# WeebLabs/DSPi

Hardware: AMD Instinct MI355X
Metric: audio samples/s (whole node), 96 kHz 11-ch 10-band PEQ; % HBM roofline (higher is better)
Workload: dtype f32

## Files before the change

dspi_amd/csrc/dspi_capi.cpp:

```cpp
#include <hip/hip_runtime.h>

#include <string.h>

#include <memory>
#include <new>
#include <cstdlib>
#include <string>
#include <unordered_map>
#include <type_traits>
#include <vector>
#include <thread>
#include <xmmintrin.h>
#include <algorithm>
#include <atomic>
#include <chrono>
#include "../../include/dspi_detmath.h"

#include "../../include/dspi.h"
#include "dspi_image.h"
#include "dspi_kernels.h"
#include "dspi_params.h"
#include "dspi_boot.h"
#include "dspi_move.h"
#include "dspi_plan.h"
#include "dspi_resize.h"
#include "dspi_snapshot.h"
#include "dspi_spdifpos.h"

using namespace dspi;

struct dspi_ctx {
    int flavor = 1;
    bool fma = false;
    uint32_t n_streams = 0, n_wg = 0;
    uint32_t cap_wg = 0;
    int device = DSPI_DEVICE_NONE;
    StateMap sm{};
    std::vector<std::unique_ptr<Params>> images;
    std::vector<uint32_t> image_refs;
    std::vector<int32_t> stream_image;
    bool assignment_dirty = true;
    bool merge_hint = false;
    std::vector<std::vector<WgItem>> image_rows;
    std::vector<uint32_t> image_rows_offset;
    PlanInput plan_in;
    LaunchPlan plan;
    WgItem *d_litems = nullptr; size_t d_litems_cap = 0;
    uint32_t *d_stream_image = nullptr; size_t d_stream_image_cap = 0;
    bool launch_dirty = true;
    uint32_t spdif_pos = 0;
    SpdifPos spdif_ps;
    uint32_t *d_spdif_ps = nullptr; size_t d_spdif_ps_cap = 0;
    uint32_t *d_spdif_vpos = nullptr; size_t d_spdif_vpos_cap = 0;
    bool populated = false;
    bool audio_started = false;
    bool no_direct = false;
    std::vector<uint32_t> lv_alphas; uint32_t lv_checked_count = 0; size_t lv_checked_n = 0;
    uint32_t direct_spin_us = 0;
    uint64_t direct_stats[5] = {0, 0, 0, 0, 0};
    hipStream_t hs = nullptr;
    hipStream_t hs_in = nullptr, hs_out = nullptr;
    std::vector<hipEvent_t> pipe_events;
    uint32_t *d_state = nullptr, *d_dlines = nullptr, *d_ring = nullptr;
    uint32_t *d_xwords = nullptr; size_t d_xwords_cap = 0;
    DevImage *d_images = nullptr;
    std::vector<uint32_t> image_flags;
    std::vector<uint8_t> image_touched;
    float *d_vals = nullptr; size_t d_vals_cap = 0;
    uint32_t *d_pv_rows = nullptr; size_t d_pv_rows_cap = 0;
    size_t d_images_cap = 0;
    WgItem *d_items = nullptr;
    size_t d_items_cap = 0;
    void *d_in = nullptr; size_t d_in_cap = 0;
    int32_t *d_pairs = nullptr; size_t d_pairs_cap = 0;
    int32_t *d_sub = nullptr; size_t d_sub_cap = 0;
    uint16_t *d_peaks = nullptr; size_t d_peaks_cap = 0;
    uint16_t *d_clip = nullptr; size_t d_clip_cap = 0;
    char *h_direct = nullptr; char *d_direct = nullptr; size_t direct_cap = 0;
    uint32_t *h_done = nullptr; uint32_t *d_done = nullptr; uint32_t direct_seq = 0; int direct_flag = -1;
    int32_t *d_spdif_words = nullptr; size_t d_spdif_words_cap = 0;
    uint32_t *d_pdm = nullptr;
    int32_t *d_pdm_in = nullptr; size_t d_pdm_in_cap = 0;
    uint32_t *d_pdm_out = nullptr; size_t d_pdm_out_cap = 0;
    int32_t *d_spdif_in = nullptr; size_t d_spdif_in_cap = 0;
    uint32_t *d_spdif_out = nullptr; size_t d_spdif_out_cap = 0;
    uint32_t *d_snap = nullptr; size_t d_snap_cap = 0;
    uint32_t *d_snap_shift = nullptr; size_t d_snap_shift_cap = 0;
    std::vector<uint8_t> active; uint32_t n_paused = 0;
    std::vector<std::pair<uint32_t, uint32_t>> paused_runs; bool paused_runs_dirty = false;
    uint32_t *d_active = nullptr; size_t d_active_cap = 0; bool active_dirty = false;
    uint32_t move_batch = 0;
    uint32_t *d_move = nullptr; size_t d_move_cap = 0;
    uint32_t *h_move = nullptr; size_t h_move_cap = 0; hipEvent_t ev_move = nullptr;
    std::string err;
};

namespace {

int fail(dspi_ctx *c, int code, const std::string &msg) { if (c) c->err = msg; return code; }

#define HIPCK(c, call)                                                                                   \
    do {                                                                                                 \
        hipError_t e_ = (call);                                                                          \
        if (e_ != hipSuccess) return fail((c), DSPI_E_HIP, std::string(#call) + ": " + hipGetErrorString(e_)); \
    } while (0)

bool valid_stream(const dspi_ctx *c, int32_t s) { return s == DSPI_ALL_STREAMS || (s >= 0 && (uint32_t)s < c->n_streams); }

int32_t add_image(dspi_ctx *c, std::unique_ptr<Params> p) {
// ... 332 lines not shown
    return 0;
}

int fetch_status(dspi_ctx *c, int32_t stream, uint16_t *peaks, uint16_t *clip) {
    for (int i = 0; i < kMaxCh; i++) peaks[i] = 0;
    *clip = 0;
    if (c->device == DSPI_DEVICE_NONE) return 0;
    const uint32_t s = stream == DSPI_ALL_STREAMS ? 0u : (uint32_t)stream;
    uint32_t w[kMaxCh + 4];
    int rc = read_stream_words(c, s, c->sm.peaks, c->sm.n_ch + 4, w);
    if (rc) return rc;
    for (int i = 0; i < c->sm.n_ch; i++) peaks[i] = (uint16_t)w[i];
    *clip = (uint16_t)(w[c->sm.n_ch] | w[c->sm.n_ch + 1] | w[c->sm.n_ch + 2] | w[c->sm.n_ch + 3]);
    return 0;
}

int zero_clips(dspi_ctx *c, int32_t stream) {
    if (c->device == DSPI_DEVICE_NONE) return 0;
    HIPCK(c, hipSetDevice(c->device));
    HIPCK(c, hipStreamSynchronize(c->hs));
    const size_t row = (size_t)c->sm.row, pitch = (size_t)c->sm.n_slots * row * 4;
    if (stream == DSPI_ALL_STREAMS) {
        HIPCK(c, hipMemset2D(c->d_state + (size_t)c->sm.clip * row, pitch, 0, 4 * row * 4, c->n_wg));
    } else {
        const uint32_t wg = (uint32_t)stream / (uint32_t)row, col = (uint32_t)stream % (uint32_t)row;
        uint32_t z[4] = {0, 0, 0, 0};
        HIPCK(c, hipMemcpy2D(c->d_state + ((size_t)wg * c->sm.n_slots + c->sm.clip) * row + col, row * 4, z, 4, 4, 4, hipMemcpyHostToDevice));
    }
    return 0;
}

}

extern "C" {

int dspi_abi_version(void) { return DSPI_ABI_VERSION; }

int dspi_create(dspi_ctx **out, int flavor, uint32_t n_streams, int hip_device) {
    const bool fma = (flavor & DSPI_FLOAT_CONTRACT_FMA) != 0, populated = (flavor & DSPI_BOOT_POPULATED_FLASH) != 0;
    flavor &= ~(DSPI_FLOAT_CONTRACT_FMA | DSPI_BOOT_POPULATED_FLASH);
    if (!out || (flavor != DSPI_FLAVOR_RP2040_Q28 && flavor != DSPI_FLAVOR_RP2350_F32) || n_streams == 0) return DSPI_E_INVAL;
    if (fma && flavor != DSPI_FLAVOR_RP2350_F32) return DSPI_E_INVAL;
    dspi_ctx *c = new (std::nothrow) dspi_ctx();
    if (!c) return DSPI_E_NOMEM;
    c->flavor = flavor;
    c->n_streams = n_streams;
    c->device = hip_device;
    c->sm = make_state_map(flavor);
    c->n_wg = (n_streams + (uint32_t)c->sm.row - 1) / (uint32_t)c->sm.row;
    c->cap_wg = c->n_wg;
    c->fma = fma;
    c->populated = populated;
    c->no_direct = getenv("DSPI_NO_DIRECT") != nullptr;
    if (const char *e = getenv("DSPI_DIRECT_SPIN_US")) { const long v = atol(e); if (v > 0) c->direct_spin_us = (uint32_t)std::min<long>(v, 1000000L); }
    if (const char *e = getenv("DSPI_MOVE_BATCH")) { const long v = atol(e); if (v > 0) c->move_batch = (uint32_t)std::min<long>(std::max<long>(v, 2L), 65535L); }
    c->images.push_back(std::make_unique<Params>(flavor, fma, !populated));
    c->image_refs.push_back(n_streams);
    c->stream_image.assign(n_streams, 0);
    *out = c;
    if (hip_device == DSPI_DEVICE_NONE) return DSPI_OK;

    int count = 0;
    if (hipGetDeviceCount(&count) != hipSuccess || count <= 0) { *out = nullptr; delete c; return DSPI_E_NODEVICE; }
    auto bail = [&](int code) { dspi_destroy(c); *out = nullptr; return code; };
    if (hipSetDevice(hip_device) != hipSuccess) return bail(DSPI_E_NODEVICE);
    if (hipStreamCreateWithFlags(&c->hs, hipStreamNonBlocking) != hipSuccess) return bail(DSPI_E_HIP);
    const size_t row = (size_t)c->sm.row;
    const size_t state_b = (size_t)c->n_wg * c->sm.n_slots * row * 4;
    const size_t dl_b = (size_t)c->n_wg * c->sm.n_out * (size_t)c->sm.max_delay * row * 4;
    const size_t ring_b = (size_t)c->n_wg * kRingLen * 2 * row * 4;
    if (hipMalloc((void **)&c->d_state, state_b) != hipSuccess || hipMalloc((void **)&c->d_dlines, dl_b) != hipSuccess ||
        hipMalloc((void **)&c->d_ring, ring_b) != hipSuccess)
        return bail(DSPI_E_NOMEM);
    if (hipMemsetAsync(c->d_state, 0, state_b, c->hs) != hipSuccess || hipMemsetAsync(c->d_dlines, 0, dl_b, c->hs) != hipSuccess ||
        hipMemsetAsync(c->d_ring, 0, ring_b, c->hs) != hipSuccess || launch_state_init(flavor, c->d_state, c->n_wg, c->hs) != hipSuccess ||
        hipStreamSynchronize(c->hs) != hipSuccess)
        return bail(DSPI_E_HIP);
    return DSPI_OK;
}

void dspi_destroy(dspi_ctx *c) {
    if (!c) return;
    if (c->device != DSPI_DEVICE_NONE) {
        (void)hipSetDevice(c->device);
        if (c->hs) (void)hipStreamSynchronize(c->hs);
        for (void *p : {(void *)c->d_state, (void *)c->d_dlines, (void *)c->d_ring, (void *)c->d_xwords, (void *)c->d_vals, (void *)c->d_pv_rows, (void *)c->d_images, (void *)c->d_items, (void *)c->d_litems, (void *)c->d_stream_image, (void *)c->d_pdm, (void *)c->d_pdm_in, (void *)c->d_pdm_out, (void *)c->d_spdif_in, (void *)c->d_spdif_out, (void *)c->d_spdif_ps, (void *)c->d_spdif_vpos, (void *)c->d_snap, (void *)c->d_snap_shift, (void *)c->d_active, (void *)c->d_move, c->d_in,
                        (void *)c->d_pairs, (void *)c->d_sub, (void *)c->d_peaks, (void *)c->d_clip, (void *)c->d_spdif_words})
            if (p) (void)hipFree(p);
        if (c->h_direct) (void)hipHostFree(c->h_direct);
        if (c->h_done) (void)hipHostFree(c->h_done);
        if (c->h_move) (void)hipHostFree(c->h_move);
        if (c->ev_move) (void)hipEventDestroy(c->ev_move);
        for (hipEvent_t e : c->pipe_events) (void)hipEventDestroy(e);
        if (c->hs_in) (void)hipStreamDestroy(c->hs_in);
        if (c->hs_out) (void)hipStreamDestroy(c->hs_out);
        if (c->hs) (void)hipStreamDestroy(c->hs);
    }
    delete c;
}

const char *dspi_last_error(const dspi_ctx *c) { return c ? c->err.c_str() : "null context"; }
int dspi_num_channels(const dspi_ctx *c) { return c ? c->sm.n_ch : DSPI_E_INVAL; }
int dspi_num_outputs(const dspi_ctx *c) { return c ? c->sm.n_out : DSPI_E_INVAL; }
int dspi_num_pairs(const dspi_ctx *c) { return c ? c->sm.n_pairs : DSPI_E_INVAL; }
uint32_t dspi_num_streams(const dspi_ctx *c) { return c ? c->n_streams : 0; }
uint32_t dspi_tile_streams(const dspi_ctx *c) { return c ? (uint32_t)c->sm.row : 0; }
// ... 57 lines not shown
        if (cap < 1) return DSPI_E_SHORT;
        const uint8_t slot = wValue & 0xFF, type = (wValue >> 8) & 0xFF;
        bool changes = false;
        for (size_t i = 0; i < c->images.size() && !changes; i++) {
            if (stream == DSPI_ALL_STREAMS ? c->image_refs[i] == 0 : (size_t)c->stream_image[(size_t)stream] != i) continue;
            const Params &r = *c->images[i];
            changes = slot < r.n_pairs && type <= 1 && type != r.output_types[slot];
        }
        if (!changes) { Params view = readable(c, stream); return view.vendor_get(req, wValue, buf, cap, peaks, &clip); }
    }
    if (req == 0xD6 || req == 0xC0) {
        return for_targets(c, stream, [&](Params &p) { int r = p.vendor_get(req, wValue, buf, cap, peaks, &clip); return r < 0 ? r : 0; }) == 0 ? 1 : DSPI_E_SHORT;
    }
    Params tmp_view = readable(c, stream);
    n = tmp_view.vendor_get(req, wValue, buf, cap, peaks, &clip);
    if (req == 0x83 && n >= 0 && (before != 0 || stream == DSPI_ALL_STREAMS)) { int rc = zero_clips(c, stream); if (rc) return rc; }
    return n;
}
int dspi_set_host_volume(dspi_ctx *c, int32_t stream, int16_t v) {
    return for_targets(c, stream, [&](Params &p) { p.set_volume(v); return 0; });
}
int dspi_set_mute(dspi_ctx *c, int32_t stream, int mute) {
    return for_targets(c, stream, [&](Params &p) { p.set_mute(mute != 0); return 0; });
}
int dspi_set_sample_rate(dspi_ctx *c, int32_t stream, uint32_t hz) {
    if (hz != 44100 && hz != 48000 && hz != 96000) return DSPI_E_INVAL;
    return for_targets(c, stream, [&](Params &p) { return p.set_rate(hz); });
}

int dspi_get_status(dspi_ctx *c, int32_t stream, void *buf, size_t cap) {
    if (!c || !buf || !valid_stream(c, stream)) return DSPI_E_INVAL;
    const int n = c->sm.n_ch * 2 + 4;
    if (cap < (size_t)n) return DSPI_E_SHORT;
    return dspi_vendor_get(c, stream, 0x50, 9, buf, (uint16_t)n);
}
int dspi_clear_clips(dspi_ctx *c, int32_t stream) {
    if (!c || !valid_stream(c, stream)) return DSPI_E_INVAL;
    uint16_t f = 0;
    int n = dspi_vendor_get(c, stream, 0x83, 0, &f, 2);
    return n < 0 ? n : (int)f;
}

int dspi_debug_image(dspi_ctx *c, int32_t stream, void *buf, size_t cap) {
    if (!c || !buf || !valid_stream(c, stream)) return DSPI_E_INVAL;
    if (cap < sizeof(DevImage)) return DSPI_E_SHORT;
    DevImage img;
    readable(c, stream).build_image(img);
    memcpy(buf, &img, sizeof(img));
    return (int)sizeof(img);
}

int dspi_debug_launch_plan(dspi_ctx *c, uint32_t *counts, size_t n_counts) {
    if (!c || !counts || n_counts < 5) return DSPI_E_INVAL;
    const int n = n_counts >= 7 ? 7 : n_counts >= 6 ? 6 : 5;
    uint32_t all[7] = {};
    for (const PathInfo &pi : kPaths) {
        const uint32_t k = (uint32_t)c->plan.items[(int)pi.path].size();
        all[(int)pi.group] += k;
        if (pi.paired) all[6] += k;
    }
    for (int k = 0; k < n; k++) counts[k] = all[k];
    return n;
}

int dspi_debug_direct_stats(dspi_ctx *c, uint64_t *out, size_t n) {
    if (!c || !out || n < 5) return DSPI_E_INVAL;
    for (int i = 0; i < 5; i++) out[i] = c->direct_stats[i];
    return 5;
}

int dspi_debug_image_count(dspi_ctx *c) {
    if (!c) return DSPI_E_INVAL;
    if (c->merge_hint) merge_images(c);
    return (int)c->images.size();
}

int dspi_debug_eq_taps(dspi_ctx *c, int32_t stream, int channel, const float *x, uint32_t n, float *taps, float *other) {
    if (!c || !x || !taps || !other || n == 0 || n > (1u << 20) || !valid_stream(c, stream) || stream < 0) return DSPI_E_INVAL;
    if (c->flavor != DSPI_FLAVOR_RP2350_F32 || channel < 0 || channel >= c->sm.n_ch) return DSPI_E_INVAL;
    if (c->device == DSPI_DEVICE_NONE) return fail(c, DSPI_E_NODEVICE, "host-only context: the HIP path is the only audio path");
    HIPCK(c, hipSetDevice(c->device));
    DevImage img;
    readable(c, stream).build_image(img);
    DevImage *d_img = nullptr; float *d_x = nullptr, *d_t = nullptr, *d_o = nullptr;
    const size_t nb = (size_t)n * sizeof(float);
    auto done = [&](int rc) { (void)hipFree(d_img); (void)hipFree(d_x); (void)hipFree(d_t); (void)hipFree(d_o); return rc; };
    if (hipMalloc((void **)&d_img, sizeof img) != hipSuccess || hipMalloc((void **)&d_x, nb) != hipSuccess ||
        hipMalloc((void **)&d_t, nb * (kBands + 1)) != hipSuccess || hipMalloc((void **)&d_o, nb * kBands) != hipSuccess)
        return done(fail(c, DSPI_E_NOMEM, "hipMalloc failed (EQ taps)"));
    if (hipMemcpy(d_img, &img, sizeof img, hipMemcpyHostToDevice) != hipSuccess || hipMemcpy(d_x, x, nb, hipMemcpyHostToDevice) != hipSuccess ||
        launch_eq_taps(c->fma, d_img, channel, d_x, n, d_t, d_o, c->hs) != hipSuccess || hipStreamSynchronize(c->hs) != hipSuccess ||
        hipMemcpy(taps, d_t, nb * (kBands + 1), hipMemcpyDeviceToHost) != hipSuccess || hipMemcpy(other, d_o, nb * kBands, hipMemcpyDeviceToHost) != hipSuccess)
        return done(fail(c, DSPI_E_HIP, "EQ taps failed"));
    return done(DSPI_OK);
}

int dspi_debug_detmath(dspi_ctx *c, int which, const float *a, const float *b, uint32_t n, float *out) {
    if (!c || !a || !out || ((which == 1 || which == 4) && !b) || n == 0 || n > (1u << 24) || which < 0 || which > 4) return DSPI_E_INVAL;
    if (c->device == DSPI_DEVICE_NONE) return fail(c, DSPI_E_NODEVICE, "host-only context: the HIP path is the only audio path");
    HIPCK(c, hipSetDevice(c->device));
    float *d_a = nullptr, *d_b = nullptr, *d_o = nullptr;
    const size_t nb = (size_t)n * sizeof(float);
    auto done = [&](int rc) { (void)hipFree(d_a); (void)hipFree(d_b); (void)hipFree(d_o); return rc; };
    if (hipMalloc((void **)&d_a, nb) != hipSuccess || hipMalloc((void **)&d_b, nb) != hipSuccess || hipMalloc((void **)&d_o, nb) != hipSuccess)
        return done(fail(c, DSPI_E_NOMEM, "hipMalloc failed (detmath)"));
    if (hipMemcpy(d_a, a, nb, hipMemcpyHostToDevice) != hipSuccess || hipMemcpy(d_b, (which == 1 || which == 4) ? b : a, nb, hipMemcpyHostToDevice) != hipSuccess ||
        launch_detmath(which, d_a, d_b, n, d_o, c->hs) != hipSuccess || hipStreamSynchronize(c->hs) != hipSuccess ||
        hipMemcpy(out, d_o, nb, hipMemcpyDeviceToHost) != hipSuccess)
// ... 796 lines not shown
            if ((he = hipEventRecord(c->pipe_events[2 * ch], sin)) != hipSuccess || (he = hipStreamWaitEvent(c->hs, c->pipe_events[2 * ch], 0)) != hipSuccess) return fail_hip(he, "event");
        }
        if ((rc = launch_rows(c, a, L, r0, r1))) { unpin(); return rc; }
        if (n_chunks > 1) {
            if ((he = hipEventRecord(c->pipe_events[2 * ch + 1], c->hs)) != hipSuccess || (he = hipStreamWaitEvent(sout, c->pipe_events[2 * ch + 1], 0)) != hipSuccess) return fail_hip(he, "event");
        }
        for (int k = 1; k < 4; k++)
            if (bufs[k].host && (he = copy(bufs[k], hipMemcpyDeviceToHost, sout)) != hipSuccess) return fail_hip(he, bufs[k].what);
    }
    if (clip_out) {
        if ((rc = gather_clip(c, c->d_clip))) { unpin(); return rc; }
        if ((he = hipMemcpyAsync(clip_out, c->d_clip, L.clip.bytes, hipMemcpyDeviceToHost, c->hs)) != hipSuccess) return fail_hip(he, "D2H clip flags");
    }
    if (n_chunks > 1) {
        if ((he = hipStreamSynchronize(c->hs_out)) != hipSuccess) return fail_hip(he, "sync");
        if ((he = hipStreamSynchronize(c->hs_in)) != hipSuccess) return fail_hip(he, "sync");
    }
    if ((he = hipStreamSynchronize(c->hs)) != hipSuccess) return fail_hip(he, "sync");
    unpin();
    return DSPI_OK;
}

int dspi_process(dspi_ctx *c, const void *pcm_in, int bit_depth, uint32_t n_blocks, uint32_t block_len, const dspi_out *out, uint32_t flags) {
    if (!c || !pcm_in || !out) return DSPI_E_INVAL;
    constexpr uint32_t kKnownFlags = DSPI_MEM_DEVICE | DSPI_OUT_TILED | DSPI_OUT_ENABLED_ONLY | DSPI_OUT_I2S_SLOTS | DSPI_OUT_SPDIF | DSPI_OUT_CLIP_FLAGS;
    if (flags & ~kKnownFlags) return fail(c, DSPI_E_INVAL, "dspi_process: undefined flag bits");
    if (c->device == DSPI_DEVICE_NONE) return fail(c, DSPI_E_NODEVICE, "host-only context: the HIP path is the only audio path");
    if ((bit_depth != 16 && bit_depth != 24) || n_blocks == 0 || block_len == 0 || block_len > DSPI_MAX_BLOCK_LEN)
        return fail(c, DSPI_E_INVAL, "bit_depth must be 16/24, 1 <= block_len <= 192, n_blocks >= 1");
    const auto call_t0 = std::chrono::steady_clock::now();
    HIPCK(c, hipSetDevice(c->device));
    int rc = commit_params(c);
    if (rc || (rc = check_leveller_alphas(c, block_len))) return rc;

    uint16_t *const clip_out = (flags & DSPI_OUT_CLIP_FLAGS) ? out->clip_flags : nullptr;
    CallInput in;
    in.n_streams = c->n_streams; in.n_wg = c->n_wg; in.row = (uint32_t)c->sm.row; in.n_ch = (uint32_t)c->sm.n_ch; in.n_out = (uint32_t)c->sm.n_out;
    in.n_pairs = (uint32_t)c->sm.n_pairs; in.n_blocks = n_blocks; in.block_len = block_len; in.bit_depth = (uint32_t)bit_depth; in.flags = flags;
    in.pairs = out->pairs; in.sub = out->sub; in.peaks = out->peaks; in.clip = clip_out; in.no_direct = c->no_direct;
    in.all_latency = c->flavor != 0; in.spdif_per_stream = c->spdif_ps.on;
    for (const PathInfo &pi : kPaths)
        if (pi.group != PathGroup::Latency && !c->plan.items[(int)pi.path].empty()) in.all_latency = false;
    const CallLayout L = plan_call(in);
    const bool tiled = flags & DSPI_OUT_TILED, spdif = flags & DSPI_OUT_SPDIF;
    if (spdif && (tiled || (flags & DSPI_OUT_I2S_SLOTS))) return fail(c, DSPI_E_INVAL, "DSPI_OUT_SPDIF goes with neither DSPI_OUT_TILED nor DSPI_OUT_I2S_SLOTS");
    if (L.spdif_two_pass && c->spdif_ps.on && (rc = upload_spdif_pos(c))) return rc;

    KArgs a{};
    a.img = c->d_images; a.stream_image = c->d_stream_image; a.vals = c->d_vals;
    a.state = c->d_state; a.dlines = c->d_dlines; a.ring = c->d_ring;
    a.n_streams = c->n_streams; a.n_blocks = n_blocks; a.block_len = block_len; a.bit_depth = (uint32_t)bit_depth;
    a.tiled_out = tiled ? 1u : 0u;
    a.fma = c->fma ? 1u : 0u;
    a.skip_silent = ((flags & DSPI_OUT_ENABLED_ONLY) && !L.spdif_two_pass) ? 1u : 0u;
    a.i2s_slots = (flags & DSPI_OUT_I2S_SLOTS) ? 1u : 0u;
    if (spdif) { a.spdif = L.spdif_two_pass ? 0u : 1u; a.spdif_pos = c->spdif_pos; }
    if (c->flavor && !tiled) {
        const size_t xb = (size_t)c->n_wg * 3 * kMaxOut * kChunk * c->sm.row * 4;
        if ((rc = ensure(c, c->d_xwords, c->d_xwords_cap, xb))) return rc;
        a.xwords = c->d_xwords;
    }

    switch (L.mem) {
    case CallMem::Device: rc = process_device(c, L, a, pcm_in, out, clip_out); break;
    case CallMem::Direct: rc = process_direct(c, L, a, pcm_in, out, clip_out, flags, call_t0); break;
    case CallMem::Staged: rc = process_staged(c, L, a, pcm_in, out, clip_out, flags); break;
    }
    if (rc == DSPI_OK && spdif) {
        c->spdif_pos = (uint32_t)((c->spdif_pos + L.frames) % 192u);
        if (c->spdif_ps.on) c->spdif_ps.advance(L.frames);
    }
    return rc;
}

}
```

dspi_amd/csrc/dspi_chain_pk.inc:

```

typedef float v2f __attribute__((ext_vector_type(2)));
typedef uint32_t v2u __attribute__((ext_vector_type(2)));

#ifndef DSPI_EXP_EMIT
#define DSPI_EXP_EMIT 0
#endif
#ifndef DSPI_EMIT_PAIRS
#define DSPI_EMIT_PAIRS 0xC
#endif
constexpr uint32_t ROWP = 128;
constexpr int HALF = 64;
constexpr int kMailbox = 8;

__device__ __forceinline__ v2f as_v2f(v2u u) { return __builtin_bit_cast(v2f, u); }
__device__ __forceinline__ v2u as_v2u(v2f f) { return __builtin_bit_cast(v2u, f); }
__device__ __forceinline__ v2f splat(float f) { return v2f{f, f}; }
__device__ __forceinline__ float clamp_pm1(float x) {
    float r;
    asm("v_med3_f32 %0, %1, -1.0, 1.0" : "=v"(r) : "v"(x));
    return r;
}
__device__ __forceinline__ float peak_acc(float pk, float x) { asm("v_max_f32 %0, |%1|, %0" : "+v"(pk) : "v"(x)); return pk; }
__device__ __forceinline__ float peak_acc2(float pk, float a, float b) { asm("v_max3_f32 %0, |%1|, |%2|, %0" : "+v"(pk) : "v"(a), "v"(b)); return pk; }

// ... 1002 lines not shown
    constexpr int P = make_state_map(1).n_pairs;
    const size_t F = (size_t)g.n_blocks * g.B;
    const int en = TAIL ? (int)min((uint32_t)T, g.B - e_cq * T) : T;
    uint32_t stream_ = stream, lane_ = lane;
    asm volatile("" : "+v"(stream_), "+v"(lane_));
    if (e_cq == 0) { pk[0] = splat(0.0f); pk[1] = splat(0.0f); }
#pragma unroll
    for (int side = 0; side < 2; ++side)
#pragma unroll
        for (int i = 0; i < T; i += 2) {
            const v2f y0 = live(dl[side][i], TAIL, i, en), y1 = live(dl[side][i + 1], TAIL, i + 1, en);
            pk[side].x = peak_acc2(pk[side].x, y0.x, y1.x);
            pk[side].y = peak_acc2(pk[side].y, y0.y, y1.y);
        }
    if (e_cq == g.cpb - 1) {
#pragma unroll
        for (int side = 0; side < 2; ++side) {
            const int oo = 2 * p + side;
            v2u p16;
#pragma unroll
            for (int c = 0; c < 2; ++c) {
                p16[c] = (uint32_t)(fminf(1.0f, pk[side][c]) * 32767.0f);
                if (pk[side][c] > 1.001f) clip[c] |= 1u << (2 + oo);
                if (a.peaks) a.peaks[((size_t)(stream_ + c) * g.n_blocks + e_kq) * sm.n_ch + 2 + oo] = (uint16_t)p16[c];
            }
            if (e_kq == g.n_blocks - 1) *reinterpret_cast<v2u *>(a.state + ((size_t)wg * sm.n_slots + sm.peaks + 2 + oo) * ROWP + lane_ * 2) = p16;
        }
    }
    if (a.pairs) {
        const float scale = ((img->out_enabled >> (2 * p)) & 3u) ? 8388607.0f : 0.0f;
        const bool shift = a.i2s_slots && ((img->i2s_pairs >> p) & 1u);
        int32_t *dst0 = a.pairs + (((size_t)(stream_ - a.pairs_stream0) * P + p) * F + (size_t)e_kq * g.B + (size_t)e_cq * T) * 2;
        int32_t *dst1 = dst0 + (size_t)P * F * 2;
        auto word = [&](v2f y) {
            const v2f d = v2f{clamp_pm1(y.x), clamp_pm1(y.y)} * scale;
            v2u w = v2u{(uint32_t)(int32_t)d.x, (uint32_t)(int32_t)d.y};
            if (shift) w = w << 8u;
            return w;
        };
#pragma unroll
        for (int j = 0; j < T / 2; ++j) {
            const v2u l0 = word(dl[0][2 * j]), r0 = word(dl[1][2 * j]);
            if (!TAIL || 2 * j + 1 < en) {
                const v2u l1 = word(dl[0][2 * j + 1]), r1 = word(dl[1][2 * j + 1]);
                st4(dst0 + j * 4, u32x4{l0.x, r0.x, l1.x, r1.x});
                st4(dst1 + j * 4, u32x4{l0.y, r0.y, l1.y, r1.y});
            } else if (2 * j < en) {
                *reinterpret_cast<v2u *>(dst0 + j * 4) = v2u{l0.x, r0.x};
                *reinterpret_cast<v2u *>(dst1 + j * 4) = v2u{l0.y, r0.y};
            }
        }
    }
}
constexpr int emit_pair_count(unsigned m) { return m ? 1 + emit_pair_count(m & (m - 1)) : 0; }
constexpr int emit_pair_nth(unsigned m, int n) { return n == 0 ? __builtin_ctz(m | 0x100u) : emit_pair_nth(m & (m - 1), n - 1); }

struct PkRole { int kind, o; };
__device__ __forceinline__ PkRole pk_role(int r) {
    const int grp = r / 3, k = r % 3;
    if (grp == 0) return {k, 0};
    return {3, (grp - 1) + 3 * k};
}
constexpr int kPkWaves = 12;

template <bool TAIL, bool LEV, bool PCM24, bool TILED, bool FMA, bool PV = false, bool PVB = false>
__global__ __launch_bounds__(64 * kPkWaves, 1) void chain_kernel_pk(KArgs a) {
    constexpr StateMap sm = make_state_map(1);
    extern __shared__ __attribute__((aligned(16))) uint32_t lds[];
    v2f *lds_state = reinterpret_cast<v2f *>(lds);
    v2f *lds_pk = lds_state + sm.lds_slots * HALF;
    v2f *xch = lds_pk + sm.n_ch * HALF;
    v2f *mailbox = xch + 2 * 2 * T * HALF;

    const WgItem item = a.items[blockIdx.x];
    const uint32_t wg = item.wg;
    const uint32_t lane = threadIdx.x & 63u;
    const int wave = __builtin_amdgcn_readfirstlane((int)(threadIdx.x >> 6));
    const uint32_t stream = wg * ROWP + lane * 2;
    asm volatile("s_mov_b64 exec, %0" ::"s"(item.mask) : "memory");
    ImgPtr img = to_const(a.img + item.image);
    const float *tile = PV ? a.vals + (size_t)wg * kPvTileFloats : nullptr;

    uint32_t *gs = a.state + (size_t)wg * sm.n_slots * ROWP + lane * 2;
    v2u *lds2 = reinterpret_cast<v2u *>(lds);
    for (int s = wave; s < sm.lds_slots; s += kPkWaves) lds2[s * HALF + lane] = *reinterpret_cast<const v2u *>(gs + (size_t)s * ROWP);
    uint32_t *role_cnt = reinterpret_cast<uint32_t *>(mailbox + kMailbox * HALF);
    v2f *envpost = mailbox + kMailbox * HALF + 2;
    const uint32_t first_lane = (uint32_t)__builtin_ctzll(item.mask);
    if (wave == 0 && lane == first_lane) { role_cnt[0] = 0; role_cnt[1] = 0; role_cnt[2] = 0; role_cnt[3] = 0; }
    __syncthreads();
    const uint32_t simd = (__builtin_amdgcn_s_getreg(4 | (4 << 6) | (1 << 11))) & 3u;
    uint32_t slot = 0;
    if (lane == first_lane) slot = atomicAdd(&role_cnt[simd], 1u);
    slot = __builtin_amdgcn_readlane(slot, first_lane);
    __syncthreads();
    uint32_t rank = slot;
    for (uint32_t q = 0; q < simd; ++q) rank += role_cnt[q];
    rank = __builtin_amdgcn_readfirstlane(rank);
    auto ld2 = [&](int slot) { return *reinterpret_cast<const v2u *>(gs + (size_t)slot * ROWP); };
    auto st2 = [&](int slot, v2u v) { *reinterpret_cast<v2u *>(gs + (size_t)slot * ROWP) = v; };

    Geo g;
    g.n_blocks = a.n_blocks; g.B = a.block_len;
    g.cpb = (g.B + T - 1) / T;
    g.items = g.n_blocks * g.cpb;
    g.lag = LEV ? (g.cpb > 3u ? g.cpb : 3u) : 0u;
// ... 82 lines not shown
            if constexpr (PVB) {
                if (split && decide) {
                    m.env_r = envpost[(2 + (kd & 1u)) * HALF + lane];
                    pv_gain_decision<FMA>(tile, lane, m, envpost[(kd & 1u) * HALF + lane], g.B, mailbox, kd);
                    decide = false;
                }
            }
            if (st >= g.lag && st < g.items + g.lag) {
                master_handoff_pk<TAIL, FMA, PV>(a, img, tile, sm, g, m, xl, xr, xch, mailbox, wg, lane, stream, true, kq, cq, st - g.lag);
                if (++cq == g.cpb) { cq = 0; ++kq; }
            }
            if (PVB && split && st < g.items) { if (++c1 == g.cpb) { decide = true; kd = k1; c1 = 0; ++k1; } }
            if (st + 1 >= g.lag && st + 1 < g.items + g.lag) master_fetch_pk<TAIL>(img, g, m, xl, xr, ring, ring_r, lane, cq);
            WT_BEFORE_BARRIER;
            lds_barrier();
            WT_AFTER_BARRIER;
        }
        WT_FINISH(rank);
        st2(sm.xfeed + 0, as_v2u(m.lpL)); st2(sm.xfeed + 1, as_v2u(m.lpR));
        st2(sm.xfeed + 2, as_v2u(m.apL)); st2(sm.xfeed + 3, as_v2u(m.apR));
        st2(sm.clip + 0, m.clip);
        if (split) { st2(sm.lev + 2, as_v2u(m.gsm_db)); st2(sm.lev + 3, as_v2u(m.g_cur)); st2(sm.lev + 4, as_v2u(m.g_prev)); }
    } else if (role.kind == 2 && PVB && LEV) {
        bool rsplit = false;
        if constexpr (PVB && LEV) rsplit = (pv_differ(tile, 0, 2 * kBands) | pv_differ(tile, kMaxCh * kBands, 2)) != 0u;
        MasterPk m;
        m.env_l = splat(0.0f); m.env_r = splat(0.0f);
        m.rp1 = v2u{0u, 0u};
        if (rsplit) { m.env_r = as_v2f(ld2(sm.lev + 1)); m.rp1 = ld2(sm.ring_pos) & (uint32_t)(kRingLen - 1); }
        v2f xr[T];
#pragma unroll
        for (int i = 0; i < T; ++i) xr[i] = splat(0.0f);
        uint32_t k1 = 0, c1 = 0;
        WT_DECL;
        for (uint32_t st = 0; st < g.steps; ++st) {
            if constexpr (PVB && LEV) {
                if (rsplit) {
                    if (st < g.items) {
                        master_intake_pv<TAIL, PCM24, FMA>(a, img, tile, sm, g, m, xr, lds_state, mailbox, envpost, ring, ring_r, lane, stream, k1, c1, 2);
                        if (++c1 == g.cpb) { c1 = 0; ++k1; }
                    } else {
                        asm volatile("s_waitcnt vmcnt(0)" ::: "memory");
                    }
                }
            }
            WT_BEFORE_BARRIER;
            lds_barrier();
            WT_AFTER_BARRIER;
        }
        WT_FINISH(rank);
        if (rsplit) st2(sm.lev + 1, as_v2u(m.env_r));
    } else if (role.kind == 2 && ext_emit) {
        constexpr int NP = emit_pair_count(ext_mask);
        v2u widx_e = ld2(sm.widx), clip = v2u{0u, 0u};
        v2f pk[NP > 0 ? NP : 1][2];
#pragma unroll
        for (int j = 0; j < NP; ++j) { pk[j][0] = splat(0.0f); pk[j][1] = splat(0.0f); }
        uint32_t e_kq = 0, e_cq = 0;
        asm volatile("" : "+v"(widx_e));
        const uint32_t dmask = (uint32_t)sm.max_delay - 1u;
        WT_DECL;
        for (uint32_t st = 0; st < g.steps; ++st) {
            const uint32_t q = st - g.lag - 1;
            if (st >= g.lag + 3 && q - 2u < g.items) {
                v2f dl[NP > 0 ? NP : 1][2][T];
                if (NP > 0) pair_emit_load<TAIL>(a, img, sm, widx_e, dl[0], wg, lane, emit_pair_nth(ext_mask, 0), e_cq, q - 2u);
#pragma unroll
                for (int j = 0; j < NP; ++j) {
                    if (j + 1 < NP) pair_emit_load<TAIL>(a, img, sm, widx_e, dl[j + 1], wg, lane, emit_pair_nth(ext_mask, j + 1), e_cq, q - 2u);
                    pair_emit_finish<TAIL>(a, img, sm, g, dl[j], pk[j], clip, wg, lane, stream, emit_pair_nth(ext_mask, j), e_kq, e_cq);
                }
                if (++e_cq == g.cpb) {
                    e_cq = 0; ++e_kq;
                    if (img->flags & IF_ANY_DELAY) widx_e = (widx_e + g.B) & dmask;
                }
            }
            WT_BEFORE_BARRIER;
            lds_barrier();
            WT_AFTER_BARRIER;
        }
        WT_FINISH(rank);
        atomicOr(gs + (size_t)(sm.clip + 1) * ROWP, clip.x);
        atomicOr(gs + (size_t)(sm.clip + 1) * ROWP + 1, clip.y);
    } else if (role.kind != 3) {
        for (uint32_t st = 0; st < g.steps; ++st) lds_barrier();
    } else {
        OutPk s;
        s.widx = ld2(sm.widx);
        s.loading = ld2(sm.mute + 0); s.counter = ld2(sm.mute + 1); s.smooth = as_v2f(ld2(sm.mute + 2));
        s.vmm = splat(0.0f);
        s.clip = v2u{0u, 0u};
        s.u_pk[0] = s.u_pk[1] = splat(0.0f); s.u_w = 0u;
        const OutConst<PV> oc = load_out_const<PV>(img, tile, lane, role.o, g.B);
        if (!(xcopy && role.o != sm.n_out - 1)) s.u_w = oc.dly_k;
        uint32_t kq = 0, cq = 0, e_kq = 0, e_cq = 0, fin_k = 0;
        bool fin_prev = false;
#ifndef DSPI_NO_TOPUSE
        asm volatile("" : "+v"(s.widx), "+v"(s.loading), "+v"(s.counter), "+v"(s.smooth));
#endif
        const bool emits = xcopy && role.o != sm.n_out - 1 && !((ext_mask >> (role.o >> 1)) & 1u);
        WT_DECL;
        for (uint32_t st = 0; st < g.steps; ++st) {
            const uint32_t q = st - g.lag - 1;
            const bool work = st >= g.lag + 1 && q < g.items, emit_prev = emits && st >= g.lag + 3 && q - 2u < g.items;
            if (work || emit_prev || fin_prev) {
                output_item_pk<TAIL, TILED, FMA, PV, PVB>(a, img, tile, oc, sm, g, s, lds_state, lds_pk, xch, wg, lane, stream, role.o, kq, cq, q, work, emit_prev, e_kq, e_cq, fin_prev, fin_k);
                fin_prev = emit_prev && e_cq == g.cpb - 1; fin_k = e_kq;
                if (work && ++cq == g.cpb) { cq = 0; ++kq; }
                if (emit_prev && ++e_cq == g.cpb) { e_cq = 0; ++e_kq; }
            } else if (xcopy && role.o != sm.n_out - 1 && !emits && st == g.lag + 1 + g.items) {
                asm volatile("s_waitcnt vmcnt(0)" ::: "memory");
            }
            WT_BEFORE_BARRIER;
            lds_barrier();
            WT_AFTER_BARRIER;
        }
        WT_FINISH(rank);
        if (fin_prev) output_item_pk<TAIL, TILED, FMA, PV, PVB>(a, img, tile, oc, sm, g, s, lds_state, lds_pk, xch, wg, lane, stream, role.o, kq, cq, g.items + 2u, false, false, e_kq, e_cq, true, fin_k);
        if (role.o == 0) {
            st2(sm.widx, s.widx);
            st2(sm.mute + 0, s.loading); st2(sm.mute + 1, s.counter); st2(sm.mute + 2, as_v2u(s.smooth));
        }
        const int cslot = sm.clip + 1 + (role.o % 3);
        atomicOr(gs + (size_t)cslot * ROWP, s.clip.x);
        atomicOr(gs + (size_t)cslot * ROWP + 1, s.clip.y);
    }
    __syncthreads();
    for (int s = wave; s < sm.lds_slots; s += kPkWaves) *reinterpret_cast<v2u *>(gs + (size_t)s * ROWP) = lds2[s * HALF + lane];
}
```

dspi_amd/csrc/dspi_kernels.h:

```cpp
#pragma once
#include <hip/hip_runtime_api.h>
#include <stddef.h>
#include <stdint.h>
#include "dspi_image.h"
#include "dspi_plan.h"

namespace dspi {

constexpr int kChunk = 16;

struct KArgs {
    const DevImage *img;
    const WgItem *items;
    uint32_t *state;
    uint32_t *dlines;
    uint32_t *ring;
    const void *pcm;
    int32_t *pairs;
    int32_t *sub;
    uint16_t *peaks;
    uint32_t n_streams, n_blocks, block_len, bit_depth;
    const uint32_t *stream_image;
    uint32_t tiled_out;
    uint32_t *xwords;
    const float *vals;
    uint32_t pairs_stream0;
    uint32_t skip_silent;
    uint32_t i2s_slots;
    uint32_t spdif;
    uint32_t spdif_pos;
    uint32_t fma;
};

size_t chain_lds_bytes(int flavor, int packed);
hipError_t launch_chain(Path path, const KArgs &args, uint32_t n_items, hipStream_t stream);
hipError_t launch_state_ops(int flavor, const WgItem *items, uint32_t n_items, const StateOps &ops, uint32_t *state, uint32_t *dlines,
                            uint32_t *ring, uint32_t n_streams, hipStream_t stream);
hipError_t launch_pv_build(const DevImage *img, const uint32_t *stream_image, const uint32_t *rows, uint32_t n_rows, float *vals, uint32_t n_streams, bool all_differ,
                           const uint32_t *active, hipStream_t stream);
hipError_t launch_state_init(int flavor, uint32_t *state, uint32_t n_wg, hipStream_t stream);
hipError_t launch_eq_taps(bool fma, const DevImage *img, int ch, const float *x, uint32_t n, float *taps, float *other, hipStream_t stream);

constexpr int kPdmStateWords = 9;
constexpr int kPdmRngWord = 7;
constexpr uint32_t pdm_power_on_word(int i) { return i == kPdmRngWord ? 123456789u : 0u; }
hipError_t launch_pdm(bool tiled, uint32_t *state, const int32_t *sub, uint32_t *words, uint32_t n_streams, uint32_t n_frames, uint32_t row,
                      uint32_t n_wg, const uint32_t *active, hipStream_t stream);
hipError_t launch_pdm_reset(uint32_t *state, uint32_t n_streams, uint32_t row, uint32_t n_wg, int32_t only_stream, int init, hipStream_t stream);

struct SpdifRates { const DevImage *img; const uint32_t *stream_image; uint32_t stream0; const uint32_t *active = nullptr; };
hipError_t launch_spdif(bool tiled, const int32_t *pairs, uint32_t *out, uint32_t n_streams, uint32_t n_pairs, uint32_t n_frames, uint32_t row,
                        uint32_t n_wg, uint32_t block_pos, uint32_t fs, const SpdifRates &rates, hipStream_t stream, const uint32_t *stream_pos = nullptr);
hipError_t launch_i2s(bool tiled, const int32_t *pairs, uint32_t *out, uint32_t n_streams, uint32_t n_pairs, uint32_t n_frames, uint32_t row,
                      uint32_t n_wg, uint32_t pair_mask, hipStream_t stream);

hipError_t launch_detmath(int which, const float *a, const float *b, uint32_t n, float *out, hipStream_t stream);
hipError_t launch_clip_gather(const uint32_t *state, uint32_t n_streams, uint32_t row, uint32_t n_slots, uint32_t clip_slot, uint16_t *out, hipStream_t stream);

struct StateArrays { uint32_t *state, *dlines, *ring, *pdm; };

hipError_t launch_snapshot(int flavor, bool import, const StateArrays &arr, uint32_t *records, uint32_t first, uint32_t count, hipStream_t stream);
hipError_t launch_snapshot_realign(int flavor, const StateArrays &arr, uint32_t *records, uint32_t first, uint32_t count, uint32_t n_streams, uint32_t *shift, hipStream_t stream,
                                   const uint32_t *active = nullptr, uint32_t r_first = 0, uint32_t r_count = 0);

hipError_t launch_move_targets(int flavor, const uint32_t *state, const uint32_t *targets, uint32_t n, uint32_t *shift, hipStream_t stream);
hipError_t launch_move_gather(int flavor, const StateArrays &arr, uint32_t *records, const uint32_t *items, const uint32_t *colrec, uint32_t n_items, hipStream_t stream);
hipError_t launch_move_scatter(int flavor, const StateArrays &arr, uint32_t *records, const uint32_t *items, const uint32_t *colrec, uint32_t n_items, const uint32_t *shift,
                               hipStream_t stream);

hipError_t launch_boot(int flavor, const StateArrays &arr, const uint32_t *items, uint32_t n_items, hipStream_t stream);

}
```

dspi_amd/host.py:

```python
from __future__ import annotations

import ctypes as C
from pathlib import Path

import numpy as np

import os

LIB_PATH = Path(os.environ.get("DSPI_LIB") or (Path(__file__).resolve().parent / "csrc" / "libdspi_mi355x.so"))

ALL = -1
MEM_DEVICE = 0x1
SNAP_REALIGN = 0x100
RESUME_AS_IS = 0x1
MOVE_AS_IS = 0x1
COMPACT_ONE_WAY = 0x1
BOOT_STREAMS_AS_IS = 0x1
RESIZE_PAUSED = 0x1
OUT_TILED = 0x2
OUT_ENABLED_ONLY = 0x4
OUT_I2S_SLOTS = 0x8
OUT_SPDIF = 0x10
OUT_CLIP_FLAGS = 0x20
E_INVAL = -10
# ... 154 lines not shown
    def save_slot(self, slot_index: int = 0, stream: int = 0) -> bytes:
        buf = C.create_string_buffer(4096)
        n = self._ck(self.L.dspi_save_preset_slot(self.h, stream, buf, 4096, slot_index), "save_slot")
        return buf.raw[:n]

    def vendor_set(self, req: int, wvalue: int, payload: bytes, stream: int = ALL) -> int:
        return self.L.dspi_vendor_set(self.h, stream, req, wvalue, payload, len(payload))

    def vendor_get(self, req: int, wvalue: int, cap: int = 64, stream: int = 0):
        buf = C.create_string_buffer(max(cap, 1))
        n = self.L.dspi_vendor_get(self.h, stream, req, wvalue, buf, cap)
        return None if n < 0 else buf.raw[:n]

    def set_volume(self, v: int, stream: int = ALL):
        return self._ck(self.L.dspi_set_host_volume(self.h, stream, v), "set_host_volume")

    def set_mute(self, m: bool, stream: int = ALL):
        return self._ck(self.L.dspi_set_mute(self.h, stream, int(m)), "set_mute")

    def set_rate(self, hz: int, stream: int = ALL) -> int:
        return self.L.dspi_set_sample_rate(self.h, stream, hz)

    def status(self, stream: int = 0) -> bytes:
        n = self.C * 2 + 4
        buf = C.create_string_buffer(n)
        self._ck(self.L.dspi_get_status(self.h, stream, buf, n), "get_status")
        return buf.raw

    def clear_clips(self, stream: int = ALL) -> int:
        return self._ck(self.L.dspi_clear_clips(self.h, stream), "clear_clips")

    def debug_image(self, stream: int = 0) -> bytes:
        buf = C.create_string_buffer(8192)
        n = self._ck(self.L.dspi_debug_image(self.h, stream, buf, 8192), "debug_image")
        return buf.raw[:n]

    def spdif_block_pos(self, set: int = -1) -> int:
        return self._ck(self.L.dspi_spdif_block_pos(self.h, set), "spdif_block_pos")

    def spdif_per_stream(self, enable: int = -1) -> bool:
        return bool(self._ck(self.L.dspi_spdif_per_stream(self.h, enable), "spdif_per_stream"))

    def spdif_stream_pos(self, first: int = 0, count: int | None = None, set=None) -> np.ndarray:
        count = self.n_streams - first if count is None else count
        get = np.zeros(count, dtype=np.uint32)
        v = None
        if set is not None:
            v = np.ascontiguousarray(np.asarray(set, dtype=np.uint32).reshape(-1))
            assert len(v) == count, (len(v), count)
        self._ck(self.L.dspi_spdif_stream_pos(self.h, first, count, v.ctypes.data if v is not None else None, get.ctypes.data), "spdif_stream_pos")
        return get

    def launch_plan(self) -> dict:
        c = (C.c_uint32 * 7)()
        self._ck(min(self.L.dspi_debug_launch_plan(self.h, c, 7), 0), "debug_launch_plan")
        return dict(zip(("q28_shared", "packed_shared", "one_stream_per_lane_images", "packed_per_lane_values_and_bands", "packed_per_lane_values", "latency_layout",
                         "latency_layout_paired"), list(c)))

    def direct_stats(self) -> dict:
        c = (C.c_uint64 * 5)()
        self._ck(min(self.L.dspi_debug_direct_stats(self.h, c, 5), 0), "debug_direct_stats")
        return dict(calls=int(c[0]), blocking_waits=int(c[1]), max_enqueue_us=c[2] / 1e3, max_wait_us=c[3] / 1e3, spin_budget_us=c[4] / 1e3)

    def image_count(self) -> int:
        return self._ck(self.L.dspi_debug_image_count(self.h), "debug_image_count")

    def eq_taps(self, x: np.ndarray, channel: int, stream: int = 0):
        x = np.ascontiguousarray(x, dtype=np.float32)
        taps = np.zeros((11, x.size), dtype=np.float32); other = np.zeros((10, x.size), dtype=np.float32)
        self.L.dspi_debug_eq_taps.argtypes = [C.c_void_p, C.c_int32, C.c_int, C.c_void_p, C.c_uint32, C.c_void_p, C.c_void_p]
        self._ck(self.L.dspi_debug_eq_taps(self.h, stream, channel, x.ctypes.data, x.size, taps.ctypes.data, other.ctypes.data), "debug_eq_taps")
        return taps, other

    def tile_streams(self) -> int:
        return int(self.L.dspi_tile_streams(self.h))

    def process_host(self, pcm: np.ndarray, n_blocks: int, block_len: int, bit_depth: int = 16,
                     want_pairs=True, want_sub=True, want_peaks=True, tiled=False, out=None, enabled_only=False, i2s_slots=False, spdif=False, clip=False):
        S, F = self.n_streams, n_blocks * block_len
        pcm = np.ascontiguousarray(pcm)
        assert pcm.nbytes == S * F * (6 if bit_depth == 24 else 4), (pcm.shape, S, F)
        if out is not None:
            pairs, sub, peaks = out
            want_pairs, want_sub, want_peaks = pairs is not None, sub is not None, peaks is not None
        elif tiled:
            R = self.tile_streams(); nt = (S + R - 1) // R
            pairs = np.zeros((nt, self.P * 2, F, R), dtype=np.int32) if want_pairs else None
            sub = np.zeros((nt, F, R), dtype=np.int32) if want_sub else None
        else:
            pairs = (np.zeros((S, self.P, F, 4), dtype=np.uint32) if spdif else np.zeros((S, self.P, F, 2), dtype=np.int32)) if want_pairs else None
            sub = np.zeros((S, F), dtype=np.int32) if want_sub else None
        peaks = np.zeros((S, n_blocks, self.C), dtype=np.uint16) if want_peaks else None
        self.last_clip = np.zeros(S, dtype=np.uint16) if clip else None
        out = _Out(pairs.ctypes.data if want_pairs else None, sub.ctypes.data if want_sub else None, peaks.ctypes.data if want_peaks else None, self.last_clip.ctypes.data if clip else None)
        self._ck(self.L.dspi_process(self.h, pcm.ctypes.data, bit_depth, n_blocks, block_len, C.byref(out), (OUT_TILED if tiled else 0) | (OUT_ENABLED_ONLY if enabled_only else 0) | (OUT_I2S_SLOTS if i2s_slots else 0) | (OUT_SPDIF if spdif else 0) | (OUT_CLIP_FLAGS if clip else 0)), "process")
        return pairs, sub, peaks

    def untile(self, pairs_t: np.ndarray, sub_t: np.ndarray):
        S = self.n_streams
        pairs = sub = None
        if pairs_t is not None:
            nt, O, F, R = pairs_t.shape
            pairs = pairs_t.transpose(0, 3, 1, 2).reshape(nt * R, O // 2, 2, F).transpose(0, 1, 3, 2)[:S].copy()
        if sub_t is not None:
            nt, F, R = sub_t.shape
            sub = sub_t.transpose(0, 2, 1).reshape(nt * R, F)[:S].copy()
        return pairs, sub

    def process_device(self, pcm_ptr: int, n_blocks: int, block_len: int, bit_depth: int = 16,
                       pairs_ptr: int = 0, sub_ptr: int = 0, peaks_ptr: int = 0, tiled: bool = False, enabled_only: bool = False, i2s_slots: bool = False, spdif: bool = False,
# ... 149 lines not shown
```

Measured before the change: 360.3 billion.

## Add line-wise emitter path with 128-bit buffer loads and LDS peak meters

Adds a fast path for the emitter wave when the item mask is full and all lanes share one write index. In that path each lane reads delay-line or xword rows with 128-bit buffer loads, writes pairs with 128-bit nontemporal stores, and tracks per-column peaks by atomic max into LDS instead of in registers. Peaks are flushed at each packet end. The aim is wider, more coalesced memory access on the output path. It adds LDS atomics, extra conditions and an env switch to turn it off, and it keeps the old path as the fallback.

```diff
diff --git a/dspi_amd/csrc/dspi_capi.cpp b/dspi_amd/csrc/dspi_capi.cpp
--- a/dspi_amd/csrc/dspi_capi.cpp
+++ b/dspi_amd/csrc/dspi_capi.cpp
@@ -55,6 +55,7 @@
     bool populated = false;
     bool audio_started = false;
     bool no_direct = false;
+    bool no_emit_lines = false;
     std::vector<uint32_t> lv_alphas; uint32_t lv_checked_count = 0; size_t lv_checked_n = 0;
     uint32_t direct_spin_us = 0;
     uint64_t direct_stats[5] = {0, 0, 0, 0, 0};
@@ -493,6 +494,7 @@
     c->fma = fma;
     c->populated = populated;
     c->no_direct = getenv("DSPI_NO_DIRECT") != nullptr;
+    c->no_emit_lines = getenv("DSPI_NO_EMIT_LINES") != nullptr;
     if (const char *e = getenv("DSPI_DIRECT_SPIN_US")) { const long v = atol(e); if (v > 0) c->direct_spin_us = (uint32_t)std::min<long>(v, 1000000L); }
     if (const char *e = getenv("DSPI_MOVE_BATCH")) { const long v = atol(e); if (v > 0) c->move_batch = (uint32_t)std::min<long>(std::max<long>(v, 2L), 65535L); }
     c->images.push_back(std::make_unique<Params>(flavor, fma, !populated));
@@ -656,8 +658,9 @@
 
 int dspi_debug_launch_plan(dspi_ctx *c, uint32_t *counts, size_t n_counts) {
     if (!c || !counts || n_counts < 5) return DSPI_E_INVAL;
-    const int n = n_counts >= 7 ? 7 : n_counts >= 6 ? 6 : 5;
-    uint32_t all[7] = {};
+    const int n = n_counts >= 8 ? 8 : n_counts >= 7 ? 7 : n_counts >= 6 ? 6 : 5;
+    uint32_t all[8] = {};
+    all[7] = c->no_emit_lines ? 1u : 0u;
     for (const PathInfo &pi : kPaths) {
         const uint32_t k = (uint32_t)c->plan.items[(int)pi.path].size();
         all[(int)pi.group] += k;
@@ -1560,6 +1563,7 @@
     a.n_streams = c->n_streams; a.n_blocks = n_blocks; a.block_len = block_len; a.bit_depth = (uint32_t)bit_depth;
     a.tiled_out = tiled ? 1u : 0u;
     a.fma = c->fma ? 1u : 0u;
+    a.no_emit_lines = c->no_emit_lines ? 1u : 0u;
     a.skip_silent = ((flags & DSPI_OUT_ENABLED_ONLY) && !L.spdif_two_pass) ? 1u : 0u;
     a.i2s_slots = (flags & DSPI_OUT_I2S_SLOTS) ? 1u : 0u;
     if (spdif) { a.spdif = L.spdif_two_pass ? 0u : 1u; a.spdif_pos = c->spdif_pos; }
diff --git a/dspi_amd/csrc/dspi_chain_pk.inc b/dspi_amd/csrc/dspi_chain_pk.inc
--- a/dspi_amd/csrc/dspi_chain_pk.inc
+++ b/dspi_amd/csrc/dspi_chain_pk.inc
@@ -1078,6 +1078,85 @@
         }
     }
 }
+__device__ __forceinline__ void pair_lines_load(const KArgs &a, ImgPtr img, const StateMap &sm, uint32_t w0, u32x4 (&v)[2][2][4],
+                                                uint32_t wg, uint32_t lane, int p, uint32_t e_cq, uint32_t e_q) {
+    constexpr int N = make_state_map(1).n_out;
+    const uint32_t flags = img->flags;
+    const uint32_t dmask = (uint32_t)sm.max_delay - 1u;
+    uint32_t g8 = lane >> 3, j8 = lane & 7u;
+    asm volatile("" : "+v"(g8), "+v"(j8));
+    __amdgpu_buffer_rsrc_t rs[2];
+    uint32_t off[2][2];
+#pragma unroll
+    for (int side = 0; side < 2; ++side) {
+        const int oo = 2 * p + side;
+        const int32_t dly_ = img->delay_samples[oo];
+        const bool dl_on_ = (flags & IF_ANY_DELAY) && dly_ > 0;
+        const bool direct_ = dl_on_ && (dly_ >= sm.max_delay || dly_ <= sm.max_delay - 3 * T);
+        uint32_t *src = direct_ ? a.dlines + ((size_t)wg * N + oo) * (size_t)sm.max_delay * ROWP
+                                : a.xwords + (((size_t)wg * 3 + (e_q % 3u)) * kMaxOut + oo) * (T * ROWP);
+        rs[side] = __builtin_amdgcn_make_buffer_rsrc(src, 0, (int)((direct_ ? (uint32_t)sm.max_delay : (uint32_t)T) * ROWP * 4u), 0x00020000);
+        const uint32_t pos0 = direct_ ? w0 + e_cq * T - (uint32_t)dly_ : 0u, pm = direct_ ? dmask : (uint32_t)T - 1u;
+#pragma unroll
+        for (int e = 0; e < 2; ++e) off[side][e] = (((pos0 + 2u * j8 + (uint32_t)e) & pm) * ROWP + 4u * g8) * 4u;
+    }
+#pragma unroll
+    for (int u = 0; u < 4; ++u)
+#pragma unroll
+        for (int side = 0; side < 2; ++side)
+#pragma unroll
+            for (int e = 0; e < 2; ++e) v[side][e][u] = __builtin_amdgcn_raw_buffer_load_b128(rs[side], (int)(off[side][e] + (uint32_t)u * 128u), 0, 16);
+}
+__device__ __forceinline__ void pair_lines_finish(const KArgs &a, ImgPtr img, const Geo &g, const u32x4 (&v)[2][2][4], uint32_t *__restrict__ acc,
+                                                  uint32_t wg, uint32_t lane, int p, uint32_t e_kq, uint32_t e_cq) {
+    constexpr int P = make_state_map(1).n_pairs;
+    const size_t F = (size_t)g.n_blocks * g.B;
+    uint32_t g8 = lane >> 3, j8 = lane & 7u;
+    asm volatile("" : "+v"(g8), "+v"(j8));
+    const float scale = ((img->out_enabled >> (2 * p)) & 3u) ? 8388607.0f : 0.0f;
+    const bool shift = a.i2s_slots && ((img->i2s_pairs >> p) & 1u);
+    auto word = [&](uint32_t l, uint32_t r) {
+        const v2f d = v2f{clamp_pm1(as_f(l)), clamp_pm1(as_f(r))} * scale;
+        v2u w = v2u{(uint32_t)(int32_t)d.x, (uint32_t)(int32_t)d.y};
+        if (shift) w = w << 8u;
+        return w;
+    };
+    int32_t *dst = a.pairs ? a.pairs + (((size_t)(wg * ROWP + 4u * g8 - a.pairs_stream0) * P + p) * F + (size_t)e_kq * g.B + (size_t)e_cq * T + 2u * j8) * 2 : nullptr;
+    const size_t sstride = (size_t)P * F * 2;
+    uint32_t *m = acc + 4u * g8;
+#pragma unroll
+    for (int u = 0; u < 4; ++u)
+#pragma unroll
+        for (int k = 0; k < 4; ++k) {
+            float ml, mr;
+            asm("v_max3_f32 %0, |%1|, |%2|, 0" : "=v"(ml) : "v"(as_f(v[0][0][u][k])), "v"(as_f(v[0][1][u][k])));
+            asm("v_max3_f32 %0, |%1|, |%2|, 0" : "=v"(mr) : "v"(as_f(v[1][0][u][k])), "v"(as_f(v[1][1][u][k])));
+            atomicMax(m + (32 * u + k), as_u(ml));
+            atomicMax(m + (ROWP + 32 * u + k), as_u(mr));
+            if (dst) {
+                const v2u f0 = word(v[0][0][u][k], v[1][0][u][k]), f1 = word(v[0][1][u][k], v[1][1][u][k]);
+                __builtin_nontemporal_store(u32x4{f0.x, f0.y, f1.x, f1.y}, reinterpret_cast<u32x4 *>(dst + (size_t)(32 * u + k) * sstride));
+            }
+        }
+}
+__device__ __forceinline__ void pair_lines_packet_end(const KArgs &a, const StateMap &sm, const Geo &g, uint32_t *__restrict__ acc, v2u &clip,
+                                                      uint32_t wg, uint32_t lane, int p, uint32_t e_kq) {
+#pragma unroll
+    for (int side = 0; side < 2; ++side) {
+        const int oo = 2 * p + side;
+#pragma unroll
+        for (int h = 0; h < 2; ++h) {
+            uint32_t col = lane + 64u * (uint32_t)h;
+            asm volatile("" : "+v"(col));
+            const float pk = as_f(acc[side * ROWP + col]);
+            acc[side * ROWP + col] = 0u;
+            const uint32_t p16 = (uint32_t)(fminf(1.0f, pk) * 32767.0f);
+            if (pk > 1.001f) clip[h] |= 1u << (2 + oo);
+            if (a.peaks) a.peaks[((size_t)(wg * ROWP + col) * g.n_blocks + e_kq) * sm.n_ch + 2 + oo] = (uint16_t)p16;
+            if (e_kq == g.n_blocks - 1) a.state[((size_t)wg * sm.n_slots + sm.peaks + 2 + oo) * ROWP + col] = p16;
+        }
+    }
+}
 constexpr int emit_pair_count(unsigned m) { return m ? 1 + emit_pair_count(m & (m - 1)) : 0; }
 constexpr int emit_pair_nth(unsigned m, int n) { return n == 0 ? __builtin_ctz(m | 0x100u) : emit_pair_nth(m & (m - 1), n - 1); }
 
@@ -1266,36 +1345,76 @@
         if (rsplit) st2(sm.lev + 1, as_v2u(m.env_r));
     } else if (role.kind == 2 && ext_emit) {
         constexpr int NP = emit_pair_count(ext_mask);
-        v2u widx_e = ld2(sm.widx), clip = v2u{0u, 0u};
-        v2f pk[NP > 0 ? NP : 1][2];
-#pragma unroll
-        for (int j = 0; j < NP; ++j) { pk[j][0] = splat(0.0f); pk[j][1] = splat(0.0f); }
+        v2u widx_e = ld2(sm.widx);
         uint32_t e_kq = 0, e_cq = 0;
         asm volatile("" : "+v"(widx_e));
         const uint32_t dmask = (uint32_t)sm.max_delay - 1u;
-        WT_DECL;
-        for (uint32_t st = 0; st < g.steps; ++st) {
-            const uint32_t q = st - g.lag - 1;
-            if (st >= g.lag + 3 && q - 2u < g.items) {
-                v2f dl[NP > 0 ? NP : 1][2][T];
-                if (NP > 0) pair_emit_load<TAIL>(a, img, sm, widx_e, dl[0], wg, lane, emit_pair_nth(ext_mask, 0), e_cq, q - 2u);
-#pragma unroll
-                for (int j = 0; j < NP; ++j) {
-                    if (j + 1 < NP) pair_emit_load<TAIL>(a, img, sm, widx_e, dl[j + 1], wg, lane, emit_pair_nth(ext_mask, j + 1), e_cq, q - 2u);
-                    pair_emit_finish<TAIL>(a, img, sm, g, dl[j], pk[j], clip, wg, lane, stream, emit_pair_nth(ext_mask, j), e_kq, e_cq);
-                }
-                if (++e_cq == g.cpb) {
-                    e_cq = 0; ++e_kq;
-                    if (img->flags & IF_ANY_DELAY) widx_e = (widx_e + g.B) & dmask;
-                }
-            }
-            WT_BEFORE_BARRIER;
-            lds_barrier();
-            WT_AFTER_BARRIER;
-        }
-        WT_FINISH(rank);
-        atomicOr(gs + (size_t)(sm.clip + 1) * ROWP, clip.x);
-        atomicOr(gs + (size_t)(sm.clip + 1) * ROWP + 1, clip.y);
+        static_assert(NP * 2 * ROWP * sizeof(uint32_t) <= 2 * 2 * HALF * sizeof(v2f), "the emitter wave's LDS meters: two pairs fit the posted envelopes' area");
+        uint32_t *acc = reinterpret_cast<uint32_t *>(envpost);
+        uint32_t w0 = (uint32_t)__builtin_amdgcn_readfirstlane((int)widx_e.x);
+        const bool lines = !TAIL && !a.no_emit_lines && item.mask == ~0ull && __all(widx_e.x == widx_e.y && widx_e.x == w0) &&
+                           (!a.pairs || ((reinterpret_cast<uintptr_t>(a.pairs) & 127u) == 0 && (g.n_blocks * g.B) % 16u == 0));
+        if (lines) {
+            if constexpr (!TAIL) {
+#pragma unroll
+                for (int i = 0; i < NP * 2 * 2; ++i) acc[i * 64 + lane] = 0u;
+                v2u clip = v2u{0u, 0u};
+                WT_DECL;
+                for (uint32_t st = 0; st < g.steps; ++st) {
+                    const uint32_t q = st - g.lag - 1;
+                    if (st >= g.lag + 3 && q - 2u < g.items) {
+                        u32x4 v[NP > 0 ? NP : 1][2][2][4];
+                        if (NP > 0) pair_lines_load(a, img, sm, w0, v[0], wg, lane, emit_pair_nth(ext_mask, 0), e_cq, q - 2u);
+#pragma unroll
+                        for (int j = 0; j < NP; ++j) {
+                            if (j + 1 < NP) pair_lines_load(a, img, sm, w0, v[j + 1], wg, lane, emit_pair_nth(ext_mask, j + 1), e_cq, q - 2u);
+                            pair_lines_finish(a, img, g, v[j], acc + j * 2 * ROWP, wg, lane, emit_pair_nth(ext_mask, j), e_kq, e_cq);
+                        }
+                        if (++e_cq == g.cpb) {
+#pragma unroll
+                            for (int j = 0; j < NP; ++j) pair_lines_packet_end(a, sm, g, acc + j * 2 * ROWP, clip, wg, lane, emit_pair_nth(ext_mask, j), e_kq);
+                            e_cq = 0; ++e_kq;
+                            if (img->flags & IF_ANY_DELAY) w0 = (w0 + g.B) & dmask;
+                        }
+                    }
+                    WT_BEFORE_BARRIER;
+                    lds_barrier();
+                    WT_AFTER_BARRIER;
+                }
+                WT_FINISH(rank);
+                uint32_t *cs = a.state + ((size_t)wg * sm.n_slots + sm.clip + 1) * ROWP + lane;
+                atomicOr(cs, clip.x);
+                atomicOr(cs + 64, clip.y);
+            }
+        } else {
+            v2u clip = v2u{0u, 0u};
+            v2f pk[NP > 0 ? NP : 1][2];
+#pragma unroll
+            for (int j = 0; j < NP; ++j) { pk[j][0] = splat(0.0f); pk[j][1] = splat(0.0f); }
+            WT_DECL;
+            for (uint32_t st = 0; st < g.steps; ++st) {
+                const uint32_t q = st - g.lag - 1;
+                if (st >= g.lag + 3 && q - 2u < g.items) {
+                    v2f dl[NP > 0 ? NP : 1][2][T];
+                    if (NP > 0) pair_emit_load<TAIL>(a, img, sm, widx_e, dl[0], wg, lane, emit_pair_nth(ext_mask, 0), e_cq, q - 2u);
+#pragma unroll
+                    for (int j = 0; j < NP; ++j) {
+                        if (j + 1 < NP) pair_emit_load<TAIL>(a, img, sm, widx_e, dl[j + 1], wg, lane, emit_pair_nth(ext_mask, j + 1), e_cq, q - 2u);
+                        pair_emit_finish<TAIL>(a, img, sm, g, dl[j], pk[j], clip, wg, lane, stream, emit_pair_nth(ext_mask, j), e_kq, e_cq);
+                    }
+                    if (++e_cq == g.cpb) {
+                        e_cq = 0; ++e_kq;
+                        if (img->flags & IF_ANY_DELAY) widx_e = (widx_e + g.B) & dmask;
+                    }
+                }
+                WT_BEFORE_BARRIER;
+                lds_barrier();
+                WT_AFTER_BARRIER;
+            }
+            WT_FINISH(rank);
+            atomicOr(gs + (size_t)(sm.clip + 1) * ROWP, clip.x);
+            atomicOr(gs + (size_t)(sm.clip + 1) * ROWP + 1, clip.y);
+        }
     } else if (role.kind != 3) {
         for (uint32_t st = 0; st < g.steps; ++st) lds_barrier();
     } else {
diff --git a/dspi_amd/csrc/dspi_kernels.h b/dspi_amd/csrc/dspi_kernels.h
--- a/dspi_amd/csrc/dspi_kernels.h
+++ b/dspi_amd/csrc/dspi_kernels.h
@@ -30,6 +30,7 @@
     uint32_t spdif;
     uint32_t spdif_pos;
     uint32_t fma;
+    uint32_t no_emit_lines;
 };
 
 size_t chain_lds_bytes(int flavor, int packed);
diff --git a/dspi_amd/host.py b/dspi_amd/host.py
--- a/dspi_amd/host.py
+++ b/dspi_amd/host.py
@@ -230,10 +230,10 @@
         return get
 
     def launch_plan(self) -> dict:
-        c = (C.c_uint32 * 7)()
-        self._ck(min(self.L.dspi_debug_launch_plan(self.h, c, 7), 0), "debug_launch_plan")
+        c = (C.c_uint32 * 8)()
+        self._ck(min(self.L.dspi_debug_launch_plan(self.h, c, 8), 0), "debug_launch_plan")
         return dict(zip(("q28_shared", "packed_shared", "one_stream_per_lane_images", "packed_per_lane_values_and_bands", "packed_per_lane_values", "latency_layout",
-                         "latency_layout_paired"), list(c)))
+                         "latency_layout_paired", "emit_lines_off"), list(c)))
 
     def direct_stats(self) -> dict:
         c = (C.c_uint64 * 5)()
```

Measured after the change: 381.3 billion, median of 6. +5.8%, better.
